# lisanhu/LongReadMapper

Hardware: AMD Instinct MI355X
Metric: aligned Gbp/sec (higher is better)
Workload: dtype u8/u64 integer; 1 GPU; E. coli K-12 sized synthetic reference (4641652 bp, 5% planted repeats), 100000 x 10000 bp ont-profile reads per GPU; seed_len=20, thres=300, gact_T=320, gact_O=120, gact_W=128, reads_per_gpu=100000, read_len=10000, streams=3, sa_sampled=1, parallelism=reads sharded, index replicated (1 RCCL bcast)

## Files before the change

### longreadmapper_amd/csrc/seed_kernels.hip

```cpp
#include <hip/hip_runtime.h>
#include "seed_index_dev.h"

__global__ __launch_bounds__(256) void pack2bit_kernel(const char *__restrict__ reads, uint64_t stride,
                                                       const uint32_t *__restrict__ lens,
                                                       uint8_t *__restrict__ out, uint64_t bytes_per_read,
                                                       uint32_t chunks_per_read, uint64_t n) {
    uint64_t read = blockIdx.x / chunks_per_read;
    uint32_t chunk = blockIdx.x % chunks_per_read;
    if (read >= n) return;
    uint64_t ow = (uint64_t) chunk * 256 + threadIdx.x;
    if (ow * 4 >= bytes_per_read) return;
    uint32_t len = lens[read];
    const uint8_t *r = (const uint8_t *) reads + read * stride;
    uint64_t p = ow * 16;
    uint32_t v = 0;
    if (p + 16 <= len) {
        uint32_t w[4];
        __builtin_memcpy(w, r + p, 16);
#pragma unroll
        for (int t = 0; t < 16; ++t) v |= base_code((w[t >> 2] >> (8 * (t & 3))) & 0xffu) << (2 * t);
    } else {
        for (int t = 0; t < 16; ++t) {
            uint32_t code = (p + t < len) ? base_code(r[p + t]) : 0u;
            v |= code << (2 * t);
        }
    }
    *reinterpret_cast<uint32_t *>(out + read * bytes_per_read + ow * 4) = v;
}

template <int CTRL>
__device__ __forceinline__ uint64_t quad_perm64(uint64_t v) {
    const uint32_t lo = (uint32_t) __builtin_amdgcn_update_dpp(0, (int) (uint32_t) v, CTRL, 0xf, 0xf, true);
    const uint32_t hi = (uint32_t) __builtin_amdgcn_update_dpp(0, (int) (uint32_t) (v >> 32), CTRL, 0xf, 0xf, true);
    return (uint64_t) lo | ((uint64_t) hi << 32);
}
__device__ __forceinline__ void sd_issue_shared(const LrmIndexView &ix, const SdKey &key, ulonglong2 &a, ulonglong2 &b) {
    const uint32_t lane = __lane_id();
    if (ix.sd_f == 4) {
        const uint64_t line = quad_perm64<0x00>(key.line);
        a = *reinterpret_cast<const ulonglong2 *>(ix.sd + line * 8 + (lane & 3u) * 2);
        b = a;
    } else {
        const uint64_t line = quad_perm64<0xA0>(key.line);
        const uint64_t *src = ix.sd + line * 8 + (lane & 1u) * 4;
        a = *reinterpret_cast<const ulonglong2 *>(src);
        b = *reinterpret_cast<const ulonglong2 *>(src + 2);
    }
}
__device__ __forceinline__ int sd_finish_shared(const LrmIndexView &ix, const SdKey &key, uint64_t code, const ulonglong2 &a, const ulonglong2 &b,
                                                uint64_t &k, uint64_t &c, uint32_t *cnt) {
    uint64_t W[8];
    if (ix.sd_f == 4) {
        W[0] = quad_perm64<0x00>(a.x); W[1] = quad_perm64<0x00>(a.y);
        W[2] = quad_perm64<0x55>(a.x); W[3] = quad_perm64<0x55>(a.y);
        W[4] = quad_perm64<0xAA>(a.x); W[5] = quad_perm64<0xAA>(a.y);
        W[6] = quad_perm64<0xFF>(a.x); W[7] = quad_perm64<0xFF>(a.y);
    } else {
        const uint64_t pa = quad_perm64<0xB1>(a.x), pb = quad_perm64<0xB1>(a.y);
        const uint64_t pc = quad_perm64<0xB1>(b.x), pd = quad_perm64<0xB1>(b.y);
        const bool odd = __lane_id() & 1u;
        W[0] = odd ? pa : a.x; W[1] = odd ? pb : a.y; W[2] = odd ? pc : b.x; W[3] = odd ? pd : b.y;
        W[4] = odd ? a.x : pa; W[5] = odd ? a.y : pb; W[6] = odd ? b.x : pc; W[7] = odd ? b.y : pd;
    }
    if (cnt) cnt[0] += 1;
    return sd_search(ix, key, code, W, k, c, cnt);
}

struct __attribute__((aligned(8))) WordPair { uint64_t a, b; };

__device__ __forceinline__ uint64_t read_window(const uint64_t *__restrict__ words, uint32_t j) {
    uint32_t wi = j >> 5, sh = (j & 31) * 2;
    WordPair w;
    __builtin_memcpy(&w, words + wi, sizeof(w));
    return (w.a >> sh) | ((w.b << 1) << (63 - sh));
}

template <int SS_ITEMS, bool COUNT>
__global__ __launch_bounds__(256) void seed_search_kernel(LrmIndexView ix, const uint64_t *__restrict__ reads2,
                                                          uint64_t words_per_read,
                                                          const uint32_t *__restrict__ lens,
                                                          const uint8_t *__restrict__ decided, uint64_t n,
                                                          int seed_len, uint32_t thres, int phase_lo, int phase_hi,
                                                          uint32_t cap_q, uint32_t blocks_per_read,
                                                          uint64_t *__restrict__ rec, uint32_t *__restrict__ recq,
                                                          uint32_t *__restrict__ gcnt, uint32_t *__restrict__ ghits,
                                                          LrmDevCounters *counters) {
    __shared__ uint64_t s_rec[SS_ITEMS + 64];
    __shared__ uint32_t s_traffic[3];
    uint32_t my_cnt[2] = {0, 0}, my_seeds = 0;
    if (COUNT && threadIdx.x < 3) s_traffic[threadIdx.x] = 0;
    __shared__ uint32_t s_q[SS_ITEMS + 64];
    __shared__ uint32_t s_cnt[64], s_hits[64], s_base[64];
    const uint64_t read = blockIdx.x / blocks_per_read;
    const uint32_t chunk = blockIdx.x % blocks_per_read;
    if (read >= n) return;
    if (decided && decided[read]) return;
    const int P = seed_len + 1;
    const uint32_t np = (uint32_t) (phase_hi - phase_lo + 1);
    const uint32_t cap_pp = SS_ITEMS / np + 1;
    const uint32_t tid = threadIdx.x;
    if (tid < np) { s_cnt[tid] = 0; s_hits[tid] = 0; }
    __syncthreads();
    const uint32_t len = lens[read];
    const uint32_t jl = len > (uint32_t) seed_len ? len - (uint32_t) seed_len : 0;
    const uint64_t *words = reads2 + read * words_per_read;
    const bool dense_lanes = (uint32_t) P - np <= 1u;
    const bool shared_lines = ix.sd && seed_len == ix.sd_len && np == (uint32_t) P && phase_lo == 0;
    LrmIndexView ix_nosd = ix;
    ix_nosd.sd = nullptr;
    if (shared_lines) {
        const uint32_t lim = jl < cap_q * np ? jl : cap_q * np;
        const uint32_t np_inv = 0xFFFFFFFFu / np;
        const uint64_t smask = (1ull << (2 * seed_len)) - 1ull;
#pragma unroll 1
        for (uint32_t it = 0; it < SS_ITEMS / 256; ++it) {
            const uint32_t j = chunk * SS_ITEMS + it * 256 + tid;
            const bool have = j < lim;
            const uint32_t j0 = (uint32_t) __builtin_amdgcn_readfirstlane((int) (j & ~63u));
            if (j0 >= lim) break;
            const uint64_t *wp = words + (j0 >> 5);
            const uint64_t W0 = wp[0], W1 = wp[1], W2 = wp[2];
            const uint32_t rel = j - j0, sh = (rel & 31u) * 2u;
            const uint64_t lo = rel < 32u ? W0 : W1, hi = rel < 32u ? W1 : W2;
            const uint64_t code = have ? ((lo >> sh) | ((hi << 1) << (63 - sh))) & smask : 0ull;
            const SdKey key = sd_key_of(ix, code, j & (uint32_t) (ix.sd_f - 1));
            ulonglong2 xa, xb;
            sd_issue_shared(ix, key, xa, xb);
            uint64_t k = 0, l = 0, c = 0, rr;
            const int st = sd_finish_shared(ix, key, code, xa, xb, k, c, COUNT ? my_cnt : nullptr);
            if (!have) continue;
            if (st == 1) rr = c;
            else if (st == 0) rr = 0;
            else rr = seed_one(ix_nosd, code, seed_len, j, k, l, COUNT ? my_cnt : nullptr);
            if (COUNT) my_seeds++;
            if (rr > 0 && rr < (uint64_t) thres) {
                uint32_t q = __umulhi(j, np_inv), ph = j - q * np;
                if (ph >= np) { ++q; ph -= np; }
                if (ph >= np) { ++q; ph -= np; }
                const uint32_t slot = atomicAdd(&s_cnt[ph], 1u);
                atomicAdd(&s_hits[ph], (uint32_t) rr);
                s_rec[ph * cap_pp + slot] = k | (rr << 40);
                s_q[ph * cap_pp + slot] = q;
            }
        }
    } else {
    const uint32_t np_inv_g = 0xFFFFFFFFu / np;
#pragma unroll 1
    for (uint32_t it = 0; it < SS_ITEMS / 256; ++it) {
        const uint32_t item = chunk * SS_ITEMS + it * 256 + tid;
        uint32_t q = __umulhi(item, np_inv_g), ph = item - q * np;
        if (ph >= np) { ++q; ph -= np; }
        if (ph >= np) { ++q; ph -= np; }
        uint64_t W[6] = {0, 0, 0, 0, 0, 0};
        uint32_t jw = 0;
        if (dense_lanes) {
            const uint32_t item0 = (uint32_t) __builtin_amdgcn_readfirstlane((int) (item & ~63u));
            const uint32_t q0 = item0 / np;
            if (q0 < cap_q) {
                const uint32_t j0 = (uint32_t) phase_lo + item0 % np + q0 * (uint32_t) P;
                const uint64_t *wp = words + (j0 >> 5);
                jw = j0 & ~31u;
#pragma unroll
                for (int e = 0; e < 6; ++e) W[e] = wp[e];
            }
        }
        if (q >= cap_q) break;
        const uint32_t j = (uint32_t) phase_lo + ph + q * (uint32_t) P;
        if (j >= jl) continue;
        uint64_t win, k, l;
        if (dense_lanes) {
            const uint32_t rel = j - jw, wi = rel >> 5, sh = (rel & 31u) * 2u;
            const uint64_t lo = wi == 0 ? W[0] : wi == 1 ? W[1] : wi == 2 ? W[2] : wi == 3 ? W[3] : W[4];
            const uint64_t hi = wi == 0 ? W[1] : wi == 1 ? W[2] : wi == 2 ? W[3] : wi == 3 ? W[4] : W[5];
            win = (lo >> sh) | ((hi << 1) << (63 - sh));
        } else {
            win = read_window(words, j);
        }
        const uint64_t rr = seed_one(ix, win, seed_len, j, k, l, COUNT ? my_cnt : nullptr);
        if (COUNT) my_seeds++;
        if (rr > 0 && rr < (uint64_t) thres) {
            const uint32_t slot = atomicAdd(&s_cnt[ph], 1u);
            atomicAdd(&s_hits[ph], (uint32_t) rr);
            s_rec[ph * cap_pp + slot] = k | (rr << 40);
            s_q[ph * cap_pp + slot] = q;
        }
    }
    }
    if (COUNT) { atomicAdd(&s_traffic[0], my_seeds); atomicAdd(&s_traffic[1], my_cnt[0]); atomicAdd(&s_traffic[2], my_cnt[1]); }
    __syncthreads();
    if (COUNT && tid < 3) atomicAdd(&counters->seed_traffic[tid], (unsigned long long) s_traffic[tid]);
    if (tid < np) {
        const uint32_t c = s_cnt[tid];
        if (c) {
            const uint64_t id = read * (uint64_t) P + (uint64_t) (phase_lo + (int) tid);
            s_base[tid] = atomicAdd(&gcnt[id], c);
            atomicAdd(&ghits[id], s_hits[tid]);
        }
    }
    __syncthreads();
    const uint32_t cpp_inv = 0xFFFFFFFFu / cap_pp;
    for (uint32_t e = tid; e < np * cap_pp; e += 256) {
        uint32_t ph = __umulhi(e, cpp_inv), sl = e - ph * cap_pp;
        if (sl >= cap_pp) { ++ph; sl -= cap_pp; }
        if (sl < s_cnt[ph]) {
            const uint64_t o = (read * (uint64_t) P + (uint64_t) (phase_lo + (int) ph)) * cap_q + s_base[ph] + sl;
            rec[o] = s_rec[e];
            recq[o] = s_q[e];
        }
    }
}

__global__ __launch_bounds__(256) void seed_search_debug_kernel(LrmIndexView ix, const uint64_t *__restrict__ words,
                                                                uint32_t len, int seed_len, uint32_t cap_q,
                                                                int32_t *j_out, uint64_t *rr_out, uint64_t *k_out,
                                                                uint64_t *l_out) {
    const int P = seed_len + 1;
    uint32_t item = blockIdx.x * 256 + threadIdx.x;
    uint32_t iter = item / cap_q, q = item % cap_q;
    if (iter >= (uint32_t) P) return;
    uint32_t jl = len > (uint32_t) seed_len ? len - (uint32_t) seed_len : 0;
    uint64_t j = (uint64_t) iter + (uint64_t) q * (uint64_t) P;
    uint64_t o = (uint64_t) iter * cap_q + q;
    if (j >= jl) { j_out[o] = -1; return; }
    uint64_t win = read_window(words, (uint32_t) j);
    uint64_t k, l;
    uint64_t rr = seed_one(ix, win, seed_len, (uint32_t) j, k, l);
    j_out[o] = (int32_t) j; rr_out[o] = rr; k_out[o] = k; l_out[o] = l;
}


#define MAX_PHASES 40
__global__ __launch_bounds__(256) void decide_kernel(const LrmPhaseRes *__restrict__ phase_res,
                                                     const uint32_t *__restrict__ lens, uint64_t n,
                                                     int seed_len, int mode, uint8_t *__restrict__ decided,
                                                     lrm_entry *__restrict__ best, LrmDevCounters *counters,
                                                     uint8_t *__restrict__ phase_out) {
    uint64_t read = (uint64_t) blockIdx.x * 256 + threadIdx.x;
    if (read >= n) return;
    const int P = seed_len + 1;
    const uint64_t num_seeds = lens[read] / (uint32_t) P;
    const LrmPhaseRes *pr = phase_res + read * (uint64_t) P;
    if (mode == 0) {
        uint8_t d = 0;
        if (num_seeds > 0 && P > 1) {
            LrmPhaseRes r0 = pr[0];
            uint64_t v = r0.val1 + r0.val2;
            if (5 * v > 3 * num_seeds) {
                d = 1;
                lrm_entry e = {r0.key1, r0.val1, r0.bucket1};
                best[read] = e;
                if (phase_out) phase_out[read] = 0;
                atomicAdd(&counters->decided_phase0, 1ull);
            }
        }
        decided[read] = d;
        return;
    }
    if (mode == 1 && decided[read]) return;
    uint64_t ot_key[MAX_PHASES], ot_val[MAX_PHASES], ot_bucket[MAX_PHASES];
    int ot_n = 0;
    lrm_entry out = {0, 0, 0};
    int iter;
    for (iter = 0; iter < P; ++iter) {
        if (num_seeds > 0) {
            LrmPhaseRes r = pr[iter];
            uint64_t v = r.val1 + r.val2;
            if (5 * v > 3 * num_seeds) {
                out.key = r.key1; out.val = r.val1; out.bucket = r.bucket1;
                if (mode == 2 && iter == 0 && P > 1) atomicAdd(&counters->decided_phase0, 1ull);
                break;
            } else if (r.val1 != 0) {
                uint64_t key = r.key1, bucket = key >> 4;
                bool found = false;
                for (int t = 0; t < ot_n; ++t) {
                    if (ot_bucket[t] == bucket) {
                        found = true;
                        ot_val[t] += 1;
                        if (key < ot_key[t]) ot_key[t] = key;
                    }
                }
                if (!found) { ot_key[ot_n] = key; ot_val[ot_n] = 1; ot_bucket[ot_n] = bucket; ot_n++; }
            }
        }
    }
    if (iter >= P - 1) {
        lrm_entry t1 = {0, 0, 0};
        for (int t = 0; t < ot_n; ++t)
            if (t1.val < ot_val[t]) { t1.key = ot_key[t]; t1.val = ot_val[t]; t1.bucket = ot_bucket[t]; }
        out = t1;
    }
    best[read] = out;
    if (phase_out) phase_out[read] = (uint8_t) (iter < P ? iter : P - 1);
}


int lrm_launch_seed(lrm_index *idx, lrm_workspace *ws, const char *d_reads, uint64_t stride,
                    const uint32_t *d_lens, uint64_t n, uint32_t seed_len,
                    uint32_t thres, lrm_entry *d_best, const LrmMapTune &mt, void *stream_, uint8_t *d_phase_out) {
    hipStream_t stream = (hipStream_t) stream_;
    if (n == 0) return 0;
    const int P = (int) seed_len + 1;
    const uint32_t cap_q = ws->cap_q;
    const uint64_t wpr = ws->words_per_read;

    HIPCHK(hipMemsetAsync(ws->d_counters, 0, sizeof(LrmDevCounters), stream));
    HIPCHK(hipMemsetAsync(ws->d_hcount, 0, n * (uint64_t) P * 4, stream));
    HIPCHK(hipMemsetAsync(ws->d_cnt, 0, n * (uint64_t) P * 4, stream));
    ws->n_last = n;
    {
        uint64_t bpr = wpr * 8;
        uint32_t cpr = (uint32_t) ((bpr / 4 + 255) / 256);
        uint32_t grid;
        if (lrm_grid_1d(n * cpr, "pack2bit", &grid)) return -1;
        lrm_time_begin(ws, LRM_K_PACK2BIT, stream);
        hipLaunchKernelGGL(pack2bit_kernel, dim3(grid), dim3(256), 0, stream, d_reads, stride,
                           d_lens, (uint8_t *) ws->d_reads2, bpr, cpr, n);
        lrm_time_end(ws, stream);
    }
    uint32_t tbits = 1;
    while ((1u << tbits) < thres && tbits < 31) tbits++;
    if (((uint64_t) cap_q << tbits) > 0xffffffffull) {
        lrm_set_error("read too long for the vote order key: cap_q %u << %u bits exceeds 32 bits", cap_q, tbits);
        return -1;
    }
    bool single = false;
    {
        const volatile uint64_t *hist = reinterpret_cast<const volatile uint64_t *>(ws->h_err + 2);
        const uint64_t d0 = *hist;
        if (ws->hist_n >= 64 && d0 * 50 < ws->hist_n) single = true;
        if (mt.seed_rounds == 1 || mt.seed_rounds == 2) single = mt.seed_rounds == 1;
        if (P == 1) single = true;
    }
    for (int round = single ? 1 : 0; round < 2; ++round) {
        int lo = round == 0 || single ? 0 : 1;
        int hi = round == 0 ? 0 : P - 1;
        if (lo > hi) break;
        int np = hi - lo + 1;
        const uint8_t *dec = round == 0 || single ? nullptr : ws->d_decided;
        const uint32_t ss_items = mt.ss_items;
        uint32_t bpr = (uint32_t) (((uint64_t) np * cap_q + ss_items - 1) / ss_items);
        uint32_t grid;
        if (lrm_grid_1d(n * bpr, "seed_search", &grid)) return -1;
        lrm_time_begin(ws, LRM_K_SEED_SEARCH, stream);
        auto sk = ws->counting ? seed_search_kernel<2048, true>
                               : ss_items == 1024u ? seed_search_kernel<1024, false> : ss_items == 4096u ? seed_search_kernel<4096, false> : seed_search_kernel<2048, false>;
        if (ws->counting) bpr = (uint32_t) (((uint64_t) np * cap_q + 2047) / 2048);
        if (ws->counting) grid = (uint32_t) (n * bpr);
        hipLaunchKernelGGL(sk, dim3(grid), dim3(256), mt.ss_lds_pad, stream, idx->view,
                           ws->d_reads2, wpr, d_lens, dec, n, (int) seed_len, thres, lo, hi, cap_q, bpr,
                           ws->d_rec, ws->d_recq, ws->d_cnt, ws->d_hcount, ws->d_counters);
        lrm_time_end(ws, stream);
        const LrmVoteLaunch vl = {dec, n, seed_len, lo, hi, tbits, round, &mt};
        if (lrm_launch_vote(idx, ws, vl, stream)) return -1;
        lrm_time_begin(ws, LRM_K_DECIDE, stream);
        hipLaunchKernelGGL(decide_kernel, dim3((uint32_t) ((n + 255) / 256)), dim3(256), 0, stream, ws->d_phase,
                           d_lens, n, (int) seed_len, single ? 2 : round, ws->d_decided, d_best, ws->d_counters, d_phase_out);
        lrm_time_end(ws, stream);
    }
    HIPCHK(hipMemcpyAsync((void *) (ws->h_err + 2), &ws->d_counters->decided_phase0, 8, hipMemcpyDeviceToHost, stream));
    ws->hist_n = n;
    HIPCHK(hipGetLastError());
    return 0;
}

int lrm_launch_debug_seed(lrm_index *idx, const char *d_read, uint32_t len, uint32_t seed_len,
                          uint64_t *d_reads2, uint64_t words, int32_t *d_j, uint64_t *d_rr,
                          uint64_t *d_k, uint64_t *d_l, uint64_t cap, void *stream_) {
    hipStream_t stream = (hipStream_t) stream_;
    const uint32_t P = seed_len + 1;
    uint32_t jl = len > seed_len ? len - seed_len : 0;
    uint32_t cap_q = (jl + P - 1) / P;
    if (cap_q == 0) cap_q = 1;
    if ((uint64_t) cap_q * P > cap) { lrm_set_error("debug seed buffer too small"); return -1; }
    uint64_t bpr = words * 8;
    uint32_t cpr = (uint32_t) ((bpr / 4 + 255) / 256);
    uint32_t *d_len1 = (uint32_t *) (d_reads2 + words);
    HIPCHK(hipMemcpyAsync(d_len1, &len, sizeof(uint32_t), hipMemcpyHostToDevice, stream));
    hipLaunchKernelGGL(pack2bit_kernel, dim3(cpr), dim3(256), 0, stream, d_read, (uint64_t) 0, d_len1,
                       (uint8_t *) d_reads2, bpr, cpr, (uint64_t) 1);
    uint32_t items = cap_q * P;
    hipLaunchKernelGGL(seed_search_debug_kernel, dim3((items + 255) / 256), dim3(256), 0, stream, idx->view,
                       d_reads2, len, (int) seed_len, cap_q, d_j, d_rr, d_k, d_l);
    HIPCHK(hipGetLastError());
    return (int) cap_q;
}
```

Before: 57.98 Gbp/s.

## Streamline seed search: packed LDS atomics, incremental phase math, compile-time SD params

Merges the per-phase count and hit-sum shared atomics into a single 64-bit atomic on a packed counter. Replaces the per-hit division for the phase/quotient in the shared-lines path with an incremental update per iteration. Adds a template specialization that fixes the SD index stride and slot size as compile-time constants when the index matches them. Rewrites the final flush so each wave copies one phase's contiguous records instead of scanning every slot, which cuts wasted iterations and makes global writes coalesced. The aim is fewer LDS atomics, less integer arithmetic and less divergent store traffic. The cost is extra template instantiations and reliance on the hit sum staying within 32 bits.

```diff
diff --git a/longreadmapper_amd/csrc/seed_kernels.hip b/longreadmapper_amd/csrc/seed_kernels.hip
--- a/longreadmapper_amd/csrc/seed_kernels.hip
+++ b/longreadmapper_amd/csrc/seed_kernels.hip
@@ -75,7 +75,14 @@
     return (w.a >> sh) | ((w.b << 1) << (63 - sh));
 }
 
-template <int SS_ITEMS, bool COUNT>
+__device__ __forceinline__ void ss_append(uint64_t *s_tot, uint64_t *s_rec, uint32_t *s_q, uint32_t cap_pp, uint32_t ph, uint32_t q, uint64_t k,
+                                          uint64_t rr) {
+    const uint32_t slot = (uint32_t) atomicAdd(reinterpret_cast<unsigned long long *>(&s_tot[ph]), 1ull | (rr << 32));
+    s_rec[ph * cap_pp + slot] = k | (rr << 40);
+    s_q[ph * cap_pp + slot] = q;
+}
+
+template <int SS_ITEMS, bool COUNT, bool SD48>
 __global__ __launch_bounds__(256) void seed_search_kernel(LrmIndexView ix, const uint64_t *__restrict__ reads2,
                                                           uint64_t words_per_read,
                                                           const uint32_t *__restrict__ lens,
@@ -90,7 +97,8 @@
     uint32_t my_cnt[2] = {0, 0}, my_seeds = 0;
     if (COUNT && threadIdx.x < 3) s_traffic[threadIdx.x] = 0;
     __shared__ uint32_t s_q[SS_ITEMS + 64];
-    __shared__ uint32_t s_cnt[64], s_hits[64], s_base[64];
+    __shared__ uint64_t s_tot[64];
+    __shared__ uint32_t s_base[64];
     const uint64_t read = blockIdx.x / blocks_per_read;
     const uint32_t chunk = blockIdx.x % blocks_per_read;
     if (read >= n) return;
@@ -99,7 +107,7 @@
     const uint32_t np = (uint32_t) (phase_hi - phase_lo + 1);
     const uint32_t cap_pp = SS_ITEMS / np + 1;
     const uint32_t tid = threadIdx.x;
-    if (tid < np) { s_cnt[tid] = 0; s_hits[tid] = 0; }
+    if (tid < np) s_tot[tid] = 0;
     __syncthreads();
     const uint32_t len = lens[read];
     const uint32_t jl = len > (uint32_t) seed_len ? len - (uint32_t) seed_len : 0;
@@ -108,12 +116,22 @@
     const bool shared_lines = ix.sd && seed_len == ix.sd_len && np == (uint32_t) P && phase_lo == 0;
     LrmIndexView ix_nosd = ix;
     ix_nosd.sd = nullptr;
+    LrmIndexView ixs = ix;
+    if (SD48) { ixs.sd_f = 4; ixs.sd_slot = 8; }
     if (shared_lines) {
         const uint32_t lim = jl < cap_q * np ? jl : cap_q * np;
         const uint32_t np_inv = 0xFFFFFFFFu / np;
         const uint64_t smask = (1ull << (2 * seed_len)) - 1ull;
+        const uint32_t dq = 256u / np, dph = 256u % np;
+        uint32_t q = __umulhi(chunk * SS_ITEMS + tid, np_inv), ph = chunk * SS_ITEMS + tid - q * np;
+        if (ph >= np) { ++q; ph -= np; }
+        if (ph >= np) { ++q; ph -= np; }
 #pragma unroll 1
         for (uint32_t it = 0; it < SS_ITEMS / 256; ++it) {
+            if (it) {
+                q += dq; ph += dph;
+                if (ph >= np) { ++q; ph -= np; }
+            }
             const uint32_t j = chunk * SS_ITEMS + it * 256 + tid;
             const bool have = j < lim;
             const uint32_t j0 = (uint32_t) __builtin_amdgcn_readfirstlane((int) (j & ~63u));
@@ -123,24 +141,19 @@
             const uint32_t rel = j - j0, sh = (rel & 31u) * 2u;
             const uint64_t lo = rel < 32u ? W0 : W1, hi = rel < 32u ? W1 : W2;
             const uint64_t code = have ? ((lo >> sh) | ((hi << 1) << (63 - sh))) & smask : 0ull;
-            const SdKey key = sd_key_of(ix, code, j & (uint32_t) (ix.sd_f - 1));
+            const SdKey key = sd_key_of(ixs, code, j & (uint32_t) (ixs.sd_f - 1));
+            if (SD48) __builtin_assume(key.tb <= 32u);
             ulonglong2 xa, xb;
-            sd_issue_shared(ix, key, xa, xb);
+            sd_issue_shared(ixs, key, xa, xb);
             uint64_t k = 0, l = 0, c = 0, rr;
-            const int st = sd_finish_shared(ix, key, code, xa, xb, k, c, COUNT ? my_cnt : nullptr);
+            const int st = sd_finish_shared(ixs, key, code, xa, xb, k, c, COUNT ? my_cnt : nullptr);
             if (!have) continue;
             if (st == 1) rr = c;
             else if (st == 0) rr = 0;
             else rr = seed_one(ix_nosd, code, seed_len, j, k, l, COUNT ? my_cnt : nullptr);
             if (COUNT) my_seeds++;
             if (rr > 0 && rr < (uint64_t) thres) {
-                uint32_t q = __umulhi(j, np_inv), ph = j - q * np;
-                if (ph >= np) { ++q; ph -= np; }
-                if (ph >= np) { ++q; ph -= np; }
-                const uint32_t slot = atomicAdd(&s_cnt[ph], 1u);
-                atomicAdd(&s_hits[ph], (uint32_t) rr);
-                s_rec[ph * cap_pp + slot] = k | (rr << 40);
-                s_q[ph * cap_pp + slot] = q;
+                ss_append(s_tot, s_rec, s_q, cap_pp, ph, q, k, rr);
             }
         }
     } else {
@@ -178,34 +191,35 @@
         }
         const uint64_t rr = seed_one(ix, win, seed_len, j, k, l, COUNT ? my_cnt : nullptr);
         if (COUNT) my_seeds++;
-        if (rr > 0 && rr < (uint64_t) thres) {
-            const uint32_t slot = atomicAdd(&s_cnt[ph], 1u);
-            atomicAdd(&s_hits[ph], (uint32_t) rr);
-            s_rec[ph * cap_pp + slot] = k | (rr << 40);
-            s_q[ph * cap_pp + slot] = q;
-        }
+        if (rr > 0 && rr < (uint64_t) thres) ss_append(s_tot, s_rec, s_q, cap_pp, ph, q, k, rr);
     }
     }
     if (COUNT) { atomicAdd(&s_traffic[0], my_seeds); atomicAdd(&s_traffic[1], my_cnt[0]); atomicAdd(&s_traffic[2], my_cnt[1]); }
     __syncthreads();
     if (COUNT && tid < 3) atomicAdd(&counters->seed_traffic[tid], (unsigned long long) s_traffic[tid]);
     if (tid < np) {
-        const uint32_t c = s_cnt[tid];
+        const uint64_t tot = s_tot[tid];
+        const uint32_t c = (uint32_t) tot;
         if (c) {
             const uint64_t id = read * (uint64_t) P + (uint64_t) (phase_lo + (int) tid);
             s_base[tid] = atomicAdd(&gcnt[id], c);
-            atomicAdd(&ghits[id], s_hits[tid]);
+            atomicAdd(&ghits[id], (uint32_t) (tot >> 32));
         }
     }
     __syncthreads();
-    const uint32_t cpp_inv = 0xFFFFFFFFu / cap_pp;
-    for (uint32_t e = tid; e < np * cap_pp; e += 256) {
-        uint32_t ph = __umulhi(e, cpp_inv), sl = e - ph * cap_pp;
-        if (sl >= cap_pp) { ++ph; sl -= cap_pp; }
-        if (sl < s_cnt[ph]) {
-            const uint64_t o = (read * (uint64_t) P + (uint64_t) (phase_lo + (int) ph)) * cap_q + s_base[ph] + sl;
-            rec[o] = s_rec[e];
-            recq[o] = s_q[e];
+    const uint32_t lane = tid & 63u, wave = (uint32_t) __builtin_amdgcn_readfirstlane((int) (tid >> 6));
+    const uint32_t cnt_l = lane < np ? (uint32_t) s_tot[lane] : 0u;
+    const uint32_t base_l = lane < np && cnt_l ? s_base[lane] : 0u;
+    const bool share = np < 4u;
+    for (uint32_t ph = share ? 0u : wave; ph < np; ph += share ? 1u : 4u) {
+        const uint32_t c = (uint32_t) __builtin_amdgcn_readlane((int) cnt_l, (int) ph);
+        const uint64_t o = (read * (uint64_t) P + (uint64_t) (phase_lo + (int) ph)) * cap_q + (uint32_t) __builtin_amdgcn_readlane((int) base_l, (int) ph);
+        uint64_t *rec_o = rec + o;
+        uint32_t *recq_o = recq + o;
+        const uint32_t lb = ph * cap_pp;
+        for (uint32_t sl = share ? tid : lane; sl < c; sl += share ? 256u : 64u) {
+            rec_o[sl] = s_rec[lb + sl];
+            recq_o[sl] = s_q[lb + sl];
         }
     }
 }
@@ -342,8 +356,11 @@
         uint32_t grid;
         if (lrm_grid_1d(n * bpr, "seed_search", &grid)) return -1;
         lrm_time_begin(ws, LRM_K_SEED_SEARCH, stream);
-        auto sk = ws->counting ? seed_search_kernel<2048, true>
-                               : ss_items == 1024u ? seed_search_kernel<1024, false> : ss_items == 4096u ? seed_search_kernel<4096, false> : seed_search_kernel<2048, false>;
+        const LrmIndexView &v = idx->view;
+        const bool sd48 = v.sd && v.sd_f == 4 && v.sd_slot == 8 && 8 + 2 * (v.sd_len - 3) - v.sd_bits <= 32;
+        auto sk = ws->counting ? seed_search_kernel<2048, true, false>
+                  : sd48 ? (ss_items == 1024u ? seed_search_kernel<1024, false, true> : ss_items == 4096u ? seed_search_kernel<4096, false, true> : seed_search_kernel<2048, false, true>)
+                         : (ss_items == 1024u ? seed_search_kernel<1024, false, false> : ss_items == 4096u ? seed_search_kernel<4096, false, false> : seed_search_kernel<2048, false, false>);
         if (ws->counting) bpr = (uint32_t) (((uint64_t) np * cap_q + 2047) / 2048);
         if (ws->counting) grid = (uint32_t) (n * bpr);
         hipLaunchKernelGGL(sk, dim3(grid), dim3(256), mt.ss_lds_pad, stream, idx->view,
```

Result: faster. 58.92 Gbp/s (median of 6 runs) (+1.6%).
